# JohnsonLabJanelia/laserCalib

Hardware: AMD Instinct MI355X
Metric: LM iters/sec and residual+Jacobian Mobs/s at 16 cams x 50k points (higher is better)
Workload: dtype f32; 1 GPU; 16 cams x 50000 points per GPU, full visibility, 11-parameter cameras (800000 obs per GPU, 800000 total), full on-device Schur-complement LM iteration; cams=16, points_per_gpu=50000, camera_parameters=11, observations_total=800000, parallelism=points sharded x1, cameras replicated, collectives=none

## Files before the change

lasercalib_amd/csrc/sba_chol_blocked.hpp:

```cpp
#pragma once
#include "sba_lm_kernels.hpp"

namespace SBA_NS {

constexpr int CB = 16;
constexpr int CLD = 17;
constexpr int CBS = CB * CLD;
constexpr int CHOLB_THREADS = 512;
constexpr int CHOLB_LDS_THREADS = 512;
constexpr int CHOLB_MAX_NB = 11;

__device__ inline int cb_off(int r, int c) { return (r * (r + 1) / 2 + c) * CBS; }

__device__ inline double readlane_f64(double v, int src) {
  const int lo = __builtin_amdgcn_readlane(__double2loint(v), src);
  const int hi = __builtin_amdgcn_readlane(__double2hiint(v), src);
  return __hiloint2double(hi, lo);
}
__device__ inline double rsqrt_nr(double x) {
  const double y = __builtin_amdgcn_rsq(x);
  return y * (1.5 - 0.5 * x * y * y);
}

template <bool NEWTON = true>
// ... 206 lines not shown
  for (int ks = 0; ks < 4; ++ks) pp = Mfma<S>::mma(pt[ks], pt[ks], pp);
#pragma unroll
  for (int rg = 0; rg < 4; ++rg) d[rg] -= pp[rg];
#pragma unroll
  for (int rg = 0; rg < 4; ++rg) Pblk[(lane & 15) * L::LD + Mfma<S>::row_of(lane, rg)] = pt[rg];
#pragma unroll
  for (int rg = 0; rg < 4; ++rg) Dt[Mfma<S>::row_of(lane, rg) * L::LD + (lane & 15)] = d[rg];
  __builtin_amdgcn_wave_barrier();
}

template <int MAXNB> struct CholbShared {
  int fail;
  short rc[MAXNB * (MAXNB + 1) / 2];
  double dd[MAXNB * CB];
  double x[MAXNB * CB];
};
template <int MAXNB> struct CholbPre {
  static constexpr int BPR = CHOLB_LDS_THREADS / 128;
  static constexpr int U0 = (MAXNB + BPR - 1) / BPR;
  static constexpr int NREM = MAXNB * (MAXNB - 1) / 2;
  static constexpr int TREM = CHOLB_LDS_THREADS - 64;
  static constexpr int U1_ALL = (NREM * 128 + TREM - 1) / TREM;
  static constexpr int U1 = U1_ALL < 16 ? U1_ALL : 16;
};

template <typename S, bool NEWTON, bool PREFETCHED, int MAXNB, typename L = CholLay<S>>
__device__ __forceinline__ bool cholb_core(unsigned char* __restrict__ smem, CholbShared<MAXNB>& sh, const double* __restrict__ E, const int n,
                                           double (&c0)[CholbPre<MAXNB>::U0][2], double (&c1)[CholbPre<MAXNB>::U1][2], const int (&rc1)[CholbPre<MAXNB>::U1],
                                           const S tau, long long* __restrict__ dbg, int& nstamp) {
#define CHOL_STAMP() do { if (dbg && threadIdx.x == 0) dbg[nstamp] = clock64(); ++nstamp; } while (0)
  using Pre = CholbPre<MAXNB>;
  constexpr int BPR = Pre::BPR, U0 = Pre::U0, TREM = Pre::TREM, U1 = Pre::U1;
  constexpr bool F32 = std::is_same<S, float>::value;
  const int tid = threadIdx.x, lane = tid & 63, wid = tid >> 6;
  const int nb = (n + CB - 1) / CB;
  const int n16 = nb * CB;
  const int nblk = nb * (nb + 1) / 2;
  S* Lb = reinterpret_cast<S*>(smem);
  S* s_y = Lb + nblk * L::BS;
  S* s_a0 = s_y + n16;
  const int s4 = tid >> 7, ii0 = (tid >> 3) & 15, jp0 = tid & 7;
  auto fix = [&](int I, int J, double& v0, double& v1) {
    if (I >= n || J >= n) v0 = (I == J) ? 1.0 : 0.0;
    if (I >= n || J + 1 >= n) v1 = (I == J + 1) ? 1.0 : 0.0;
  };
  if (tid < n16) s_y[tid] = (S)sh.x[tid];
  if constexpr (PREFETCHED) {
#pragma unroll
    for (int u = 0; u < U0; ++u) fix((BPR * u + s4) * CB + ii0, 2 * jp0, c0[u][0], c0[u][1]);
    {
      const int ii = ii0, jp = jp0;
#pragma unroll
      for (int u = 0; u < U0; ++u) {
        const int r = BPR * u + s4;
        if (r < nb) {
          const int I = r * CB + ii, J = 2 * jp;
          S* dst = Lb + L::off(r, 0) + ii * L::LD + J;
          const double v0 = c0[u][0] + ((I == J && I < n) ? sh.dd[I] : 0.0), v1 = c0[u][1] + ((I == J + 1 && I < n) ? sh.dd[I] : 0.0);
          dst[0] = (S)v0;
          dst[1] = (S)v1;
          if (F32 && I == J) s_a0[I] = (S)v0;
          if (F32 && I == J + 1) s_a0[I] = (S)v1;
        }
      }
    }
    __syncthreads();
    CHOL_STAMP();
    if (wid > 0) {
#pragma unroll
      for (int u = 0; u < U1; ++u) {
// ... 165 lines not shown
        const S* col = Lb + L::off(b, tid >> 4) + (tid & 15);
        S s0 = 0, s1 = 0;
#pragma unroll
        for (int i = 0; i < CB; i += 2) { s0 += col[i * L::LD] * s_y[b * CB + i]; s1 += col[(i + 1) * L::LD] * s_y[b * CB + i + 1]; }
        s_y[tid] -= s0 + s1;
      }
      __syncthreads();
    }
    if (tid < n16) sh.x[tid] = (double)s_y[tid];
  }
  __syncthreads();
  CHOL_STAMP();
  return fail;
#undef CHOL_STAMP
}

template <typename T, int MAXNB = CHOLB_MAX_NB, int LD32 = 20>
__global__ __launch_bounds__(CHOLB_LDS_THREADS) void k_cholesky_blocked(
    const double* __restrict__ E , int C,
    LMState* __restrict__ st, double* __restrict__ D2c, const ParamSets<T> ps,
    double* __restrict__ delta_c, int n_sys ,
    const int32_t* __restrict__ tie ,
    const int32_t* __restrict__ first ,
    long long* __restrict__ dbg , int use_f32, float tau32) {
  extern __shared__ __align__(16) unsigned char smem[];
  constexpr bool PIV_NEWTON = !std::is_same<T, float>::value;
  const int n = n_sys;
  const int tid = threadIdx.x, lane = tid & 63, wid = tid >> 6;
  const double* rhs = E + (size_t)n * n;
  const double* dU = rhs + n;
  const double* gct = dU + n;
  const bool pair_ok = (n & 1) == 0;
  using Pre = CholbPre<MAXNB>;
  using L32 = CholLay<float, LD32>;
  constexpr int BPR = Pre::BPR, U0 = Pre::U0, TREM = Pre::TREM, U1 = Pre::U1;
  double c0[U0][2];
  const int nlast = n - 1;
  auto addr = [&](int I, int J) { return E + (size_t)min(I, nlast) * n + min(J, nlast - 1 + (pair_ok ? 0 : 1)); };
  const int s4 = tid >> 7, ii0 = (tid >> 3) & 15, jp0 = tid & 7;
  const int tclamp = min(tid, nlast);
  if (pair_ok) {
#pragma unroll
    for (int u = 0; u < U0; ++u) {
      const double2 t = *reinterpret_cast<const double2*>(addr((BPR * u + s4) * CB + ii0, 2 * jp0));
      c0[u][0] = t.x; c0[u][1] = t.y;
    }
  } else {
#pragma unroll
    for (int u = 0; u < U0; ++u) {
      const double* q = addr((BPR * u + s4) * CB + ii0, 2 * jp0);
      c0[u][0] = q[0]; c0[u][1] = q[(2 * jp0 + 1 < n) ? 1 : 0];
    }
  }
  double in_d = D2c[tclamp], in_u = dU[tclamp], in_r = rhs[tclamp];
  const double my_g = (tid < n) ? gct[tid] : 0.0;
  double c1[U1][2];
  int rc1[U1];
  {
    const int nb_ = (n + CB - 1) / CB;
    const int last = (nb_ * (nb_ + 1) / 2 - nb_) * 128 - 1;
    int cc = 1, base = 0;
#pragma unroll
    for (int u = 0; u < U1; ++u) {
      const int e = min(max(tid - 64, 0) + TREM * u, last);
      const int k = e >> 7;
      while (k >= base + (nb_ - cc) && cc < nb_) { base += nb_ - cc; ++cc; }
      rc1[u] = ((cc + (k - base)) << 8) | cc;
      const int I = (cc + (k - base)) * CB + ((e >> 3) & 15), J = cc * CB + 2 * (e & 7);
      if (pair_ok) {
        const double2 t = *reinterpret_cast<const double2*>(addr(I, J));
        c1[u][0] = t.x; c1[u][1] = t.y;
      } else {
        const double* q = addr(I, J);
        c1[u][0] = q[0]; c1[u][1] = q[(J + 1 < n) ? 1 : 0];
      }
    }
  }
  if (st->status >= 0) return;
  const int cur_ = ps_cur(ps, st);
  const double* __restrict__ cams = ps.cams[cur_];
  double* __restrict__ cams_new = ps.cams[cur_ ^ 1];
// ... 13 lines not shown
  const double my_xs = (tid < n) ? cams[first ? first[tid] : tid] : 0.0;

  if (tid < nblk) {
    int r = 0;
    while ((r + 1) * (r + 2) / 2 <= tid) ++r;
    sh.rc[tid] = (short)((r << 8) | (tid - r * (r + 1) / 2));
  }
  if (tid == 0) { sh.fail = 0; st->cost = E[(size_t)n * n + 3 * n]; }
  if (tid < n16) {
    double dd = 0;
    if (tid >= n) in_r = 0;
    if (tid < n) {
      double d = in_d;
      if (fresh) { d = fmax(d, in_u); D2c[tid] = d; }
      dd = lam * fmax_pos(d);
    }
    sh.x[tid] = in_r;
    sh.dd[tid] = dd;
  }
  __syncthreads();
  bool fail;
  if constexpr (MAXNB > CHOLB_MAX_NB) {
    static_assert(std::is_same<T, float>::value, "the 16-block-row kernel exists for the fp32 engine only");
    fail = cholb_core<float, false, true, MAXNB, L32>(smem, sh, E, n, c0, c1, rc1, tau32, dbg, nstamp);
    if (tid == 0) { st->chol_retry = fail ? 1 : 0; if (fail) st->chol_f64_retries += 1; }
    if (fail) return;
  } else if constexpr (std::is_same<T, float>::value) {
    if (use_f32) {
      fail = cholb_core<float, false, true, MAXNB, L32>(smem, sh, E, n, c0, c1, rc1, tau32, dbg, nstamp);
      if (fail) {
        __syncthreads();
        if (tid == 0) sh.fail = 0;
        __syncthreads();
        fail = cholb_core<double, true, false, MAXNB>(smem, sh, E, n, c0, c1, rc1, 0.0, dbg, nstamp);
        if (tid == 0) atomicAdd(&st->chol_f64_retries, 1);
      }
    } else {
      fail = cholb_core<double, PIV_NEWTON, true, MAXNB>(smem, sh, E, n, c0, c1, rc1, 0.0, dbg, nstamp);
    }
  } else {
    fail = cholb_core<double, PIV_NEWTON, true, MAXNB>(smem, sh, E, n, c0, c1, rc1, 0.0, dbg, nstamp);
  }
  double pred = 0, dx2 = 0, x2 = 0, gm = 0;
  __shared__ double s_cnew[CHOLB_LDS_THREADS];
  if (tid < ncam) {
    const double d = fail ? 0.0 : sh.x[tie ? tie[tid] : tid];
    delta_c[tid] = d;
    cams_new[tid] = my_cam + d;
    s_cnew[tid] = my_cam + d;
  }
  if (tid < n) {
    const double d = fail ? 0.0 : sh.x[tid];
    pred = 0.5 * d * (sh.dd[tid] * d - my_g);
    dx2 = d * d;
    x2 = my_xs * my_xs;
    gm = fabs(my_g);
  }
  pred = wave_sum(pred); dx2 = wave_sum(dx2); x2 = wave_sum(x2); gm = wave_max(gm);
  if (lane == 0) { s_scr[0][wid] = pred; s_scr[1][wid] = dx2; s_scr[2][wid] = x2; s_scr[3][wid] = gm; }
  __syncthreads();
  if (tid == 0) {
    double p = 0, d2 = 0, xx = 0, g = 0;
    for (int w = 0; w < CHOLB_LDS_THREADS / 64; ++w) { p += s_scr[0][w]; d2 += s_scr[1][w]; xx += s_scr[2][w]; g = fmax(g, s_scr[3][w]); }
    st->pred_c = p; st->dx2_c = d2; st->x2_c = xx; st->gmax_c = g;
// ... 206 lines not shown
```

lasercalib_amd/csrc/sba_engine.hpp:

```cpp
#pragma once
#include "sba_common.hpp"
#include "sba_lm_kernels.hpp"
#include "sba_chol_blocked.hpp"
#include "sba_chol_ll.hpp"
#include "sba_chol_big.hpp"
#include "sba_sq_kernels.hpp"
#include "sba_schur_wide.hpp"
#include "sba_schur_f64.hpp"
#include "sba_ipc.hpp"
#include "sba_covariance.hpp"
#include "sba_triangulate.hpp"
#include "sba_layout.hpp"

namespace SBA_NS {
using namespace sba_host;

constexpr int MAX_CAMS = 128;

struct Knobs {
  bool no_dense = false;
  bool no_fused64 = false;
  bool no_wide = false;
  bool wide_pw2 = false;
  bool chol_ll = true, chol_ll_all = false;
  bool chol_f32 = true;
  float chol_f32_tau = 1.1920929e-7f;
  bool chol_big_dag = true;
  int chol_big_min_n = 209;
  bool decide_kernel = false;
  bool schur_scan = false;
  bool no_bf3_pairs = false;
  double dense_min_vis = 0.0;
  bool schur_debug = false;
  int schur_debug_skip = 0;
  bool chol_debug = false;
  bool upload_debug = false;
  bool solve_debug = false;
  long long ipc_timeout_ticks = IPC_TIMEOUT_TICKS;
  bool ipc_allow_cached = false;
};

inline Knobs read_knobs() {
  Knobs k;
  auto set = [](const char* name) { return getenv(name) != nullptr; };
  k.no_dense = set("SBA_NO_DENSE");
  k.no_fused64 = set("SBA_NO_FUSED64");
  k.no_wide = set("SBA_NO_WIDE");
  k.wide_pw2 = set("SBA_WIDE_PW2");
  k.decide_kernel = set("SBA_DECIDE_KERNEL");
  k.schur_scan = set("SBA_SCHUR_SCAN");
  k.no_bf3_pairs = set("SBA_NO_BF3_PAIRS");
  k.chol_debug = set("SBA_CHOL_DEBUG");
  k.upload_debug = set("SBA_UPLOAD_DEBUG");
  k.solve_debug = set("SBA_SOLVE_DEBUG");
  k.ipc_allow_cached = set("SBA_IPC_ALLOW_CACHED");
  if (const char* e = getenv("SBA_CHOL")) { k.chol_ll = std::string(e) != "blocked"; k.chol_ll_all = std::string(e) == "ll"; }
  if (const char* e = getenv("SBA_CHOL_F32")) k.chol_f32 = atoi(e) != 0;
  if (const char* e = getenv("SBA_CHOL_F32_TAU")) { char* end = nullptr; const double v = strtod(e, &end); if (end != e && v >= 0 && v < 1) k.chol_f32_tau = (float)v; }
  if (const char* e = getenv("SBA_CHOL_BIG")) k.chol_big_dag = std::string(e) != "launches";
  if (const char* e = getenv("SBA_CHOL_BIG_MIN_N")) {
    char* end = nullptr;
    const long v = strtol(e, &end, 10);
    if (end != e && *end == 0 && v >= 0) k.chol_big_min_n = (int)std::min<long>(v, CS_MAX_NB * CB);
  }
  if (const char* e = getenv("SBA_DENSE_MIN_VIS")) { char* end = nullptr; const double v = strtod(e, &end); if (end != e && v >= 0 && v <= 1) k.dense_min_vis = v; }
  if (const char* e = getenv("SBA_SCHUR_DEBUG")) { k.schur_debug = true; k.schur_debug_skip = std::max(0, atoi(e) - 1); }
  if (const char* e = getenv("SBA_IPC_TIMEOUT_S")) {
    char* end = nullptr;
    const double sec = strtod(e, &end);
    if (end != e && sec > 0 && sec < 3600) k.ipc_timeout_ticks = (long long)(sec * 1e8);
  }
  return k;
}

struct Layout {
  int C, N;
  int64_t M;
  bool dense, masked_ok, grp_indexed;
  int ngroups, npairs;
  int ncu;
// ... 122 lines not shown
  bool has_w = false;
  bool identity_perm = true;
  bool dense = false;
  bool masked_ok = false;
  DevBuf<uint16_t> vis_mask;
  DevBuf<uint16_t> grp_mask;
  DevBuf<int32_t> grp_start;
  bool grp_indexed = false;
  DevBuf<double> gdpart;
  std::vector<int64_t> perm;
  int nblk = 0, nchunk = 0, ngroups = 0, npairs = 0;
  int n = 0;
  Knobs kn;
  Route rt;

  DevBuf<T2> uv_pm, uv_cm;
  DevBuf<T> w_pm, w_cm;
  DevBuf<int32_t> ci_pm, pi_pm, pt_start, blk_pt, pi_cm, chunk_cam, chunk_begin, chunk_end, cam_chunk_start;
  DevBuf<int32_t> pair_ga, pair_gb;
  DevBuf<int4> blk_desc;
  DevBuf<double> cams[2], pts[2];
  DevBuf<T> ptsT[2], campre[2];
  int cur = 0;
  DevBuf<double> V, gp, D2p, D2c, U, gc, Upart, bpart, E_own, scal_own, delta_c, cost_part, gmax_part, trial_part;
  DevBuf<T> slabs, pfac;
  DevBuf<T2> r_pm;
  DevBuf<T> Jc_pm, Jp_pm;
  DevBuf<LMState> d_state_buf;
  struct { LMState* p = nullptr; } d_state;
  int st_slot = 0;
  bool pending_decide = false;
  const double* pend_scal = nullptr;
  int pend_ranks = 1;
  DevBuf<double> gmax_alt;
  double* gmax_cur = nullptr;
  DevBuf<sba_lm_iter_log> d_log;
  int log_read = 0;
  int cur_at_begin = 0;
  LMState* h_state = nullptr;
  sba_lm_opts opts{};
  bool lm_active = false;
  DevBuf<double> chol_sol, chol_work, chol_W, chol_Minv, chol_Ld, chol_yv;
  DevBuf<int> chol_info;
  unsigned chol_epoch = 0;
  DevBuf<unsigned> chol_dag_flags;
  DevBuf<double> chol_Mimg;
// ... 419 lines not shown
      hipLaunchKernelGGL(k_group_index, dim3((N + 255) / 256), dim3(256), 0, stream, ci_pm.p, pt_start.p, N, ngroups, grp_mask.p,
                         grp_start.p, up_flag.p);
      int flag = 1;
      HIPCHK(hipMemcpyAsync(&flag, up_flag.p, sizeof(int), hipMemcpyDeviceToHost, stream));
      up_sync();
      grp_indexed = (flag == 0);
    }
    int ncu = 256;
    hipDeviceProp_t prop;
    if (ngroups > 1 && hipGetDeviceProperties(&prop, device) == hipSuccess && prop.multiProcessorCount > 0) ncu = prop.multiProcessorCount;
    rt = plan_route<T>(Layout{C, N, M, dense, masked_ok, grp_indexed, ngroups, npairs, ncu}, kn);
    const int ksplit = rt.ksplit;

    for (int b = 0; b < 2; ++b) {
      cams[b].alloc((size_t)C * NCP); pts[b].alloc((size_t)N * 3);
      ptsT[b].alloc((size_t)N * 3); campre[b].alloc((size_t)C * CAMPRE);
    }
    pfac.alloc((size_t)std::max(N, 1) * PF);
    V.alloc((size_t)N * 6); gp.alloc((size_t)N * 3); D2p.alloc((size_t)N * 3); D2c.alloc(n);
    U.alloc((size_t)C * NCP * NCP); gc.alloc(n); Upart.alloc((size_t)std::max(1, nchunk) * 256);
    bpart.alloc(std::max((size_t)ngroups * ksplit * GROUP_ROWS, rt.fused_wide ? (size_t)ksplit * WIDE_ROWS : (size_t)0));
    slabs.alloc(std::max((size_t)npairs * ksplit * GROUP_TILES * GROUP_TILES * 256, rt.fused_wide ? (size_t)ksplit * WIDE_SLOTS * 256 : (size_t)0));
    E_own.alloc((size_t)n * n + 3 * n + 1); scal_own.alloc(NSCAL); delta_c.alloc(n);
    const int nres_blocks = (int)((M + PM_BLOCK - 1) / PM_BLOCK);
    const int nlinp = rt.nlinp;
    if (dev_general) has_vis_mask = (C <= GROUP_CAMS);
    else {
      has_vis_mask = nodup && !vmask.empty();
      if (has_vis_mask) vis_mask.upload(vmask, stream);
    }
    if (rt.fused_ok) gdpart.alloc((size_t)ksplit * 2 * (rt.fused_wide ? WIDE_ROWS : GROUP_ROWS));
    if (rt.pairs_fold_u) gdpart.alloc((size_t)ngroups * ksplit * 2 * GROUP_ROWS);
    cost_part.alloc((size_t)std::max(std::max(std::max(std::max(nblk, nres_blocks), ksplit), nlinp), 1)); gmax_part.alloc(std::max(std::max(std::max(nblk, ksplit), nlinp), 1)); gmax_alt.alloc(std::max(std::max(std::max(nblk, ksplit), nlinp), 1));
    trial_part.alloc((size_t)4 * std::max(std::max(nblk, rt.nbs_dense), 1));
    up_lap("allocations + H2D enqueue");
    up_sync();
    up_lap("H2D completion");
    uploaded = true;
    cur = 0;
    set_params(cams_h, pts_h);
    ++up_rep.stream_syncs;
    up_lap("parameters");
    up_rep.route = dev_dense ? SBA_ROUTE_DEVICE_DENSE : dev_general ? SBA_ROUTE_DEVICE_GENERAL : SBA_ROUTE_HOST;
    up_rep.dense = dense; up_rep.masked = masked_ok; up_rep.group_indexed = grp_indexed; up_rep.identity_perm = identity_perm;
    up_rep.n_blocks = nblk; up_rep.n_chunks = nchunk;
    up_rep.seconds_total = std::chrono::duration<double>(std::chrono::steady_clock::now() - up_begin).count();
// ... 729 lines not shown
    pending_decide = false;
    gmax_cur = gmax_part.p;
    lm_active = true;
    if (!std::isfinite(c0)) { err = "Residuals are not finite in the initial point."; return SBA_ERR_NONFINITE; }
    return SBA_OK;
  }

  int lm_linearize() override {
    if (!lm_active) { err = "sba_lm_begin has not been called"; return SBA_ERR_STATE; }
    poll_clean = false;
    if (!bf3_path()) flush_decide();
    if (sq_mode()) { launch_sq_linearize(d_state.p); return SBA_OK; }
    if (fused()) return SBA_OK;
    if (!lin_pts()) {
      prof_begin(KP_LINP);
      launch_linearize_points(d_state.p);
      prof_end(KP_LINP);
    }
    if (h_state->free_cams && !rt.pairs_fold_u) { prof_begin(KP_LINC); launch_linearize_cams(d_state.p); prof_end(KP_LINC); }
    return SBA_OK;
  }

  int lm_form_reduced(double* E) override { return form_reduced(E, nullptr); }
  int form_reduced(double* E, double* Pk) {
    if (!lm_active) { err = "sba_lm_begin has not been called"; return SBA_ERR_STATE; }
    poll_clean = false;
    if (!bf3_path()) flush_decide();
    if (sq_mode()) {
      if (opts.mode == SBA_MODE_CAMS_ONLY_SQ)
        hipLaunchKernelGGL(k_sq_pack_cams, dim3(64), dim3(256), 0, stream, sq_16.p, C, d_state.p, E);
      return SBA_OK;
    }
    if (h_state->free_cams) {
      prof_begin(KP_SCHUR);
      launch_schur();
      prof_end(KP_SCHUR);
    }
    prof_begin(KP_REDUCE);
    {
      const int fc = (int)h_state->free_cams;
      const bool wide = fused() && rt.fused_wide;
      const int ntw = wide_ntw(C);
      const int nt_launch = wide ? ntw * (ntw + 1) / 2 : npairs == 1 ? GROUP_TILES * (GROUP_TILES + 1) / 2 : GROUP_TILES * GROUP_TILES;
      const int np_arg = wide ? 1 : npairs;
      const int nblocks = (fc ? 4 * nt_launch * np_arg + (n + 15) / 16 : 0) + 1;
      const int emajor_mode = wide ? 3 : ((fused() && sizeof(T) == 4) || pairs_bf3()) ? 1 : 0;
      hipLaunchKernelGGL(k_build_exchange<T>, dim3(nblocks), dim3(1024), 0, stream, slabs.p, bpart.p, rt.ksplit, pair_ga.p,
                         pair_gb.p, np_arg, U.p, gc.p, cost_part.p, n_lin_parts(), C, fc, E, d_state.p,
                         (fused() || rt.pairs_fold_u) ? gdpart.p : (const double*)nullptr, Pk, emajor_mode, nt_launch);
    }
    prof_end(KP_REDUCE);
    return SBA_OK;
  }

  void launch_chol_big(double* Esys, int n_sys, bool tied, CholRoute route) {
    const int npad = cholbig_npad(n_sys), nbr = npad / BB, nbx = (n_sys + BB - 1) / BB;
    if (chol_W.n < (size_t)npad * npad) {
      chol_W.alloc((size_t)npad * npad); chol_Minv.alloc((size_t)nbr * BB * BB); chol_Ld.alloc((size_t)nbr * BB * BB);
      chol_yv.alloc(2 * (size_t)npad);
      std::vector<long long> empty(2 * (size_t)npad, CHOLBIG_X_EMPTY);
      HIPCHK(hipMemcpyAsync(chol_yv.p, empty.data(), empty.size() * sizeof(long long), hipMemcpyHostToDevice, stream));
      sync();
    }
    if (chol_sol.n < (size_t)n_sys) { chol_sol.alloc(n_sys); chol_info.alloc(1); }
    const size_t lds = (size_t)CHOLBIG_LDS_BLOCKS * CBS * sizeof(double);
    const bool dag = route != CholRoute::BIG_LAUNCHES, dag32 = route == CholRoute::BIG_DAG_F32;
    if (dag) {
      if (chol_dag_flags.n == 0) { chol_dag_flags.alloc(choldag_nflags(CHOLDAG_MAX_NBR)); chol_dag_flags.zero(stream); }
      if (chol_Mimg.n == 0) chol_Mimg.alloc((size_t)CHOLDAG_MAX_NBR * choldag_img<double>());
      if (chol_debug) { chol_dbg.alloc(8 * (CHOLDAG_MAX_NBR + 1)); chol_dbg.zero(stream); }
      const dim3 grid(1 + nbr * (nbr + 1) / 2);
      if (dag32)
// ... 8 lines not shown
        fprintf(stderr, "[chol_dag%s, the walker, x10 ns: wait for W(c,c-1), W(c,c) | load | panel | downdate | factor+inverse | image stored | flag]\n", dag32 ? " on f32 lanes" : "");
        for (int cc = 0; cc < nbr; ++cc) {
          const long long* v = sv.data() + 8 * cc;
          fprintf(stderr, "  c=%2d at %6lld:", cc, v[4] - sv[0]);
          if (cc > 0) fprintf(stderr, " wait %4lld | load %4lld | panel %4lld | downdate %4lld |", v[1] - sv[8 * (cc - 1) + 7], v[2] - v[1], v[3] - v[2], v[4] - v[3]);
          fprintf(stderr, " factor %4lld | image %4lld | flag %4lld | column %5lld\n", v[5] - v[4], v[6] - v[5], v[7] - v[6], cc > 0 ? v[7] - sv[8 * (cc - 1) + 7] : v[7] - v[0]);
        }
        chol_debug = false;
      }
    } else {
      hipLaunchKernelGGL(k_chol_big_prepare, dim3(nbr * (nbr + 1) / 2), dim3(256), 0, stream, Esys, n_sys, d_state.p, D2c.p,
                         chol_W.p, npad, chol_info.p);
      for (int j = 0; j < nbr; ++j) {
        const int q = nbr - 1 - j;
        hipLaunchKernelGGL(k_chol_big_step, dim3(std::max(1, q * (q + 1) / 2)), dim3(CHOLBIG_THREADS), lds, stream, chol_W.p, npad, j,
                           chol_Minv.p, chol_Ld.p, chol_info.p, d_state.p);
      }
    }
    hipLaunchKernelGGL(k_chol_big_back_all<T>, dim3(nbx), dim3(256), 0, stream, (const void*)chol_W.p, npad, n_sys, chol_Ld.p, chol_Minv.p,
                       chol_yv.p, ++chol_epoch, chol_sol.p, chol_info.p, d_state.p, dag ? (const void*)chol_Mimg.p : (const void*)nullptr,
                       dag32 ? 1 : 0, Esys, C, D2c.p, ps_lm(), delta_c.p, tied ? tie_map.p : nullptr, tied ? tie_first.p : nullptr);
  }

  int lm_solve_trial(double* E, double* scal) override {
    if (!lm_active) { err = "sba_lm_begin has not been called"; return SBA_ERR_STATE; }
    poll_clean = false;
    if (opts.mode == SBA_MODE_TRANSFORM_SQ) {
      hipLaunchKernelGGL(k_sq_solve12, dim3(1), dim3(64), 0, stream, sq_16.p, d_state.p, tsets());
      launch_sq_trial();
      return SBA_OK;
    }
    if (h_state->free_cams) {
      prof_begin(KP_CHOL);
      const bool tied = (opts.mode == SBA_MODE_SHARED_INTR);
      const int n_sys = tied ? n_tied : n;
      double* Esys = E;
      if (tied) {
        hipLaunchKernelGGL(k_tie_system, dim3(n_tied), dim3(256), 0, stream, E, n, n_tied, tie_pre_start.p, tie_pre_idx.p,
                           E_tied.p, d_state.p);
        Esys = E_tied.p;
      }
      const int32_t* tie = tied ? tie_map.p : nullptr;
      const int32_t* first = tied ? tie_first.p : nullptr;
      const int nb = (n_sys + CB - 1) / CB;
      const CholRoute route = chol_route<T>(n_sys, n, kn, card_shared);
      switch (route) {
        case CholRoute::LL:
        case CholRoute::LL_F32: {
          if (chol_work.n < (size_t)nb * (nb + 1) / 2 * CB * CB) chol_work.alloc((size_t)CLL_MAX_NB * (CLL_MAX_NB + 1) / 2 * CB * CB);
          if (chol_debug && chol_dbg.n < 128) { chol_dbg.alloc(128); chol_dbg.zero(stream); }
          if constexpr (sizeof(T) == 4) {
            if (route == CholRoute::LL_F32) {
              if (nb <= 14) {
                const size_t lds32 = ((size_t)(nb * (nb + 1) / 2) * CB * 20 + 2 * (size_t)nb * CB) * sizeof(float);
                hipLaunchKernelGGL((k_cholesky_blocked<T, 16, 20>), dim3(1), dim3(CHOLB_LDS_THREADS), lds32, stream, Esys, C, d_state.p, D2c.p,
                                   ps_lm(), delta_c.p, n_sys, tie, first, (long long*)nullptr, 1, kn.chol_f32_tau);
              } else {
                const size_t lds32 = ((size_t)(nb * (nb + 1) / 2) * CB * 17 + 2 * (size_t)nb * CB) * sizeof(float);
                hipLaunchKernelGGL((k_cholesky_blocked<T, 16, 17>), dim3(1), dim3(CHOLB_LDS_THREADS), lds32, stream, Esys, C, d_state.p, D2c.p,
                                   ps_lm(), delta_c.p, n_sys, tie, first, (long long*)nullptr, 1, kn.chol_f32_tau);
              }
            }
          }
          hipLaunchKernelGGL(k_cholesky_ll<T>, dim3(1), dim3(CLL_THREADS), CLL_LDS_BYTES, stream, Esys, C, d_state.p, D2c.p,
                             ps_lm(), delta_c.p, n_sys, tie, first, chol_work.p, chol_debug ? chol_dbg.p : nullptr,
                             route == CholRoute::LL_F32 ? 1 : 0);
          if (chol_debug) {
            const std::vector<long long> st = read_stamps(chol_dbg, 128);
            if (nb > 6) {
              const long long x0 = st[2 + 2 * 3], y0 = st[3 + 2 * 3];
              fprintf(stderr, "[chol_ll step 3, cycles after the step's barrier, per wave] X done:");
              for (int w = 0; w < 8; ++w) fprintf(stderr, " %lld", st[64 + w] - x0);
              fprintf(stderr, " | Y done:");
              for (int w = 0; w < 8; ++w) fprintf(stderr, " %lld", st[72 + w] - y0);
              fprintf(stderr, "\n[chol_ll back substitution, block row 5] x done (per wave, from wave 0's):");
              for (int w = 0; w < 8; ++w) fprintf(stderr, " %lld", st[80 + w] - st[80]);
              fprintf(stderr, " | barrier passed %lld | update done:", st[96] - st[80]);
              for (int w = 0; w < 8; ++w) fprintf(stderr, " %lld", st[88 + w] - st[96]);
              fprintf(stderr, " | barrier passed %lld\n", st[97] - st[96]);
            }
            fprintf(stderr, "[chol_ll stamps, cycles] setup %lld  chol0 %lld |", st[1] - st[0], st[2] - st[1]);
            for (int j = 0; j < nb; ++j) fprintf(stderr, " X%d %lld Y%d %lld |", j, st[3 + 2 * j] - st[2 + 2 * j], j, st[4 + 2 * j] - st[3 + 2 * j]);
            fprintf(stderr, " backsub %lld  epilogue %lld  total %lld\n", st[3 + 2 * nb] - st[2 + 2 * nb], st[4 + 2 * nb] - st[3 + 2 * nb], st[4 + 2 * nb] - st[0]);
            chol_debug = false;
          }
          break;
        }
        case CholRoute::BLOCKED: {
          const size_t lds = ((size_t)(nb * (nb + 1) / 2) * CBS + 2 * (size_t)nb * CB) * sizeof(double);
          if (chol_debug && chol_dbg.n == 0) { chol_dbg.alloc(64); }
          hipLaunchKernelGGL(k_cholesky_blocked<T>, dim3(1), dim3(CHOLB_LDS_THREADS), lds, stream, Esys, C, d_state.p, D2c.p,
                             ps_lm(), delta_c.p, n_sys, tie, first, chol_debug ? chol_dbg.p : nullptr, (sizeof(T) == 4 && kn.chol_f32) ? 1 : 0,
                             kn.chol_f32_tau);
          if (chol_debug) {
            const std::vector<long long> st = read_stamps(chol_dbg, 64);
            fprintf(stderr, "[chol stamps, cycles] load %lld  chol0 %lld |", st[1] - st[0], st[2] - st[1]);
            for (int j = 0; j < nb; ++j) fprintf(stderr, " B%d %lld C%d %lld |", j, st[3 + 2 * j] - st[2 + 2 * j], j, st[4 + 2 * j] - st[3 + 2 * j]);
            fprintf(stderr, " backsub %lld  epilogue %lld  total %lld\n", st[3 + 2 * nb] - st[2 + 2 * nb], st[4 + 2 * nb] - st[3 + 2 * nb], st[4 + 2 * nb] - st[0]);
            fprintf(stderr, "[chol C0, cycles after B0's barrier, per wave]");
            for (int w = 0; w < CHOLB_LDS_THREADS / 64; ++w) fprintf(stderr, " %lld", st[40 + w] - st[3]);
            fprintf(stderr, "\n");
            chol_debug = false;
          }
          break;
        }
        case CholRoute::STREAM: {
          if (chol_sol.n < (size_t)n_sys) { chol_sol.alloc(n_sys); chol_info.alloc(1); }
          if (chol_work.n < (size_t)nb * (nb + 1) / 2 * CB * CB) chol_work.alloc((size_t)nb * (nb + 1) / 2 * CB * CB);
          const size_t fixed = ((size_t)nb * CBS + (size_t)nb * CB) * sizeof(double);
          const int scap = std::min(64, std::max(nb, (int)((150 * 1024 - fixed) / (CBS * sizeof(double)))));
          const size_t lds = fixed + (size_t)scap * CBS * sizeof(double);
          if (chol_debug && chol_dbg.n == 0) chol_dbg.alloc(64);
          hipLaunchKernelGGL(k_chol_prepare, dim3((n_sys + 255) / 256), dim3(256), 0, stream, Esys, n_sys, d_state.p, D2c.p, chol_sol.p);
          hipLaunchKernelGGL(k_cholesky_stream, dim3(1), dim3(CHOLB_THREADS), lds, stream, Esys, n_sys, chol_work.p, chol_sol.p,
                             chol_info.p, d_state.p, scap, chol_debug ? chol_dbg.p : nullptr);
          if (chol_debug) {
            const std::vector<long long> st = read_stamps(chol_dbg, 8);
            fprintf(stderr, "[chol_stream cycles] update %lld  factor %lld  solve %lld  write-back %lld  back-substitution %lld\n", st[0], st[1], st[2], st[3], st[4]);
            chol_debug = false;
          }
          hipLaunchKernelGGL(k_chol_epilogue<T>, dim3(1), dim3(1024), 0, stream, Esys, C, n_sys, d_state.p, D2c.p, ps_lm(), delta_c.p,
                             chol_sol.p, chol_info.p, tie, first);
          break;
        }
// ... 157 lines not shown
    } else {
      for (int i = 0; i < n; ++i) gmax = std::max(gmax, std::fabs(gch[i]));
    }
    if (rep) {
      const LMState& s = *h_state;
      rep->cost = cost; rep->initial_cost = initial_cost; rep->optimality = gmax; rep->step_norm = s.step_norm;
      rep->lambda = s.lam; rep->nfev = s.nfev; rep->njev = s.njev; rep->iterations = s.iter; rep->accepted = s.n_accepted;
      rep->status = s.status < 0 ? 0 : s.status;
      rep->reserved = s.chol_f64_retries;
    }
    lm_active = false;
    return SBA_OK;
  }

  int run_loop(const sba_lm_opts* o, int32_t& status, int32_t& iters) {
    int rc = SBA_OK;
    while (status < 0) {
      const int pbatch = multi() ? 2 : (bf3_path() && !kn.decide_kernel ? 2 : 1);
      int batch = prof_on ? pbatch : BATCH;
      if (o->max_iter > 0) batch = std::min(std::max(1, o->max_iter - iters), prof_on ? pbatch : 64);
      for (int b = 0; b < batch; ++b) {
        lm_linearize();
        if (!multi()) {
          lm_form_reduced(E_own.p);
          lm_solve_trial(E_own.p, nullptr);
          lm_decide_async(nullptr, 1);
        } else if (ipc_on) {
          const bool fc = h_state->free_cams != 0;
          const unsigned long long s0 = ++ipc_seq[0];
          const size_t sys_off = ipc_L.sys_slot(n, (int)(s0 & 1));
          form_reduced(E_own.p, ipc_mine + sys_off);
          ipc_publish(0, s0, d_state.p);
          ipc_gate(0, s0, d_state.p, 0, 0, nullptr);
          hipLaunchKernelGGL(k_ipc_sum_system, dim3(fc ? std::min(1024, (n * n + 255) / 256) : 1), dim3(256), 0, stream, ipc_ptrs.p, comm_n,
                             sys_off, n, (int)fc, E_own.p, d_state.p);
          const unsigned long long s1 = ++ipc_seq[1];
          const size_t sc_off = ipc_L.scal_slot((int)(s1 & 1));
          lm_solve_trial(E_own.p, ipc_mine + sc_off);
          ipc_publish(1, s1, d_state.p);
          ipc_gate(1, s1, d_state.p, sc_off, NSCAL, sc_all.p);
          lm_decide_async(sc_all.p, comm_n);
        } else {
          if (xpack.n < exch_packed_size(n)) xpack.alloc(exch_packed_size(n));
          form_reduced(E_own.p, xpack.p);
          const bool fc = h_state->free_cams != 0;
          double* xb = fc ? xpack.p : xpack.p + exch_packed_size(n) - 1;
          RCCLCHK(Rccl::get().all_reduce(xb, xb, fc ? exch_packed_size(n) : 1, Rccl::kFloat64, Rccl::kSum, comm, stream));
          hipLaunchKernelGGL(k_unpack_exchange, dim3(fc ? std::min(1024, (n * n + 255) / 256) : 1), dim3(256), 0, stream, xpack.p, n,
// ... 200 lines not shown
```

lasercalib_amd/csrc/sba_lm_kernels.hpp:

```cpp
#pragma once
#include <cstddef>
#include "sba_kernels.hpp"

namespace SBA_NS {

constexpr int CHOL_THREADS = 1024;
constexpr int CHOL_LDS_MAX_N = 176;

__host__ __device__ inline size_t exch_packed_index(int n, int i, int j) { return (size_t)i * n - (size_t)i * (i - 1) / 2 + (size_t)(j - i); }
__host__ __device__ inline size_t exch_packed_size(int n) { return (size_t)n * (n + 1) / 2 + 3 * (size_t)n + 1; }

template <typename T>
__global__ __launch_bounds__(1024) void k_build_exchange(
    const T* __restrict__ slabs, const double* __restrict__ bpart, int ksplit, const int32_t* __restrict__ pair_ga,
    const int32_t* __restrict__ pair_gb, int npairs, const double* __restrict__ U, const double* __restrict__ gc,
    const double* __restrict__ cost_part, int n_cost_part, int C, int free_cams, double* __restrict__ E,
    const LMState* __restrict__ st,
    const double* __restrict__ gdpart ,
    double* __restrict__ Pk = nullptr ,
    int emajor_mode = 0 ,
    int nt_launch = GROUP_TILES * GROUP_TILES ) {
  using M_ = Mfma<T>;
  constexpr int EPB = 64, NG = 1024 / EPB, BPT = 256 / EPB;
  __shared__ double s_p[NG][EPB];
  const int st_status = st->status;
  __shared__ double scr[16];
  constexpr int NT = GROUP_TILES * GROUP_TILES;
  const int n = C * NCP;
  const int tile_blocks = free_cams ? BPT * nt_launch * npairs : 0;
  const int row_blocks = free_cams ? (n + 15) / 16 : 0;
  const int g = threadIdx.x / EPB, l16 = threadIdx.x & (EPB - 1);
  int bid = blockIdx.x;
  if (bid < tile_blocks) {
    const bool wide = emajor_mode == 3;
    const int pair = wide ? 0 : bid / (BPT * nt_launch);
    const int rem = bid - pair * BPT * nt_launch;
    const int t = rem / BPT, part = rem - t * BPT;
    const int ga = pair_ga[pair], gb = pair_gb[pair];
    const bool diag = wide || (ga == gb);
    const int ntw = wide_ntw(C);
    const int ntile = wide ? ntw * (ntw + 1) / 2 : diag ? (GROUP_TILES * (GROUP_TILES + 1)) / 2 : NT;
    if (t >= ntile) return;
    int R, Tc;
    if (wide) wide_tile_rc(ntw, t, R, Tc);
// ... 25 lines not shown
      for (; k + 3 * NG < ksplit; k += 4 * NG) {
        s0 += (double)src[(size_t)k * stride];
        s1 += (double)src[(size_t)(k + NG) * stride];
        s2 += (double)src[(size_t)(k + 2 * NG) * stride];
        s3 += (double)src[(size_t)(k + 3 * NG) * stride];
      }
      for (; k < ksplit; k += NG) s0 += (double)src[(size_t)k * stride];
    }
    const int ci_ = i / NCP, cj_ = j / NCP;
    s_p[g][l16] = (s0 + s1) + (s2 + s3);
    __syncthreads();
    if (st_status >= 0) return;
    if (g == 0 && i < n && j < n) {
      double s = 0;
#pragma unroll
      for (int q = 0; q < NG; ++q) s += s_p[q][l16];
      double v = -s;
      if (!gdpart && ci_ == cj_) v += U[(size_t)ci_ * NCP * NCP + (i - ci_ * NCP) * NCP + (j - cj_ * NCP)];
      const bool sym_tile = diag && R == Tc;
      if (!emajor) {
        E[(size_t)i * n + j] = v;
        if (!sym_tile) E[(size_t)j * n + i] = v;
        if (Pk && i <= j) Pk[exch_packed_index(n, i, j)] = v;
      } else if (!sym_tile || i <= j) {
        E[(size_t)i * n + j] = v;
        E[(size_t)j * n + i] = v;
        if (Pk) Pk[exch_packed_index(n, i < j ? i : j, i < j ? j : i)] = v;
      }
    }
    return;
  }
  bid -= tile_blocks;
  double* rhs = E + (size_t)n * n;
  double* dU = rhs + n;
  double* gv = dU + n;
  if (bid < row_blocks) {
    constexpr int RB = 16, RG = 1024 / RB;
    __shared__ double s_r[3][RG][RB];
    const int lr = threadIdx.x & (RB - 1), gr = threadIdx.x / RB;
    const int i = bid * RB + lr;
    double b0 = 0, g0 = 0, d0 = 0;
    if (i < n) {
      const bool wide = emajor_mode == 3;
      const int rstride = wide ? WIDE_ROWS : GROUP_ROWS;
      const int grp = wide ? 0 : i / GROUP_ROWS, rho = i - grp * GROUP_ROWS;
      const double* src = bpart + (size_t)grp * ksplit * GROUP_ROWS + rho;
      if (gdpart) {
        const double* gs_ = gdpart + (size_t)grp * ksplit * 2 * GROUP_ROWS + rho;
        for (int k = gr; k < ksplit; k += RG) {
          b0 += src[(size_t)k * rstride];
// ... 554 lines not shown
```

Measured before the change: 7356 Mobs/s (observations x LM iterations per second, whole job).

## Write fp32 blocked-lower image in exchange build and load it in Cholesky

The exchange-matrix build kernel now also writes an fp32 copy of the reduced camera system, already laid out as 16x16 lower-triangular blocks. The blocked Cholesky kernel then loads whole blocks as float4 per wave from this image, instead of gathering fp64 pairs from the dense row-major E and converting them. The diagonal is rebuilt from E's diagonal plus damping, and padding is pre-initialised to identity on the host. This is meant to cut the load and convert phase of the single-block Cholesky. In exchange it adds extra scattered stores in the build kernel and a new buffer.

New measurement: 7494 Mobs/s (observations x LM iterations per second, whole job), median of 6. +1.9%, better.

```diff
diff --git a/lasercalib_amd/csrc/sba_chol_blocked.hpp b/lasercalib_amd/csrc/sba_chol_blocked.hpp
--- a/lasercalib_amd/csrc/sba_chol_blocked.hpp
+++ b/lasercalib_amd/csrc/sba_chol_blocked.hpp
@@ -252,16 +252,26 @@
   static constexpr int TREM = CHOLB_LDS_THREADS - 64;
   static constexpr int U1_ALL = (NREM * 128 + TREM - 1) / TREM;
   static constexpr int U1 = U1_ALL < 16 ? U1_ALL : 16;
+  static constexpr int PU0 = (MAXNB + CHOLB_LDS_THREADS / 64 - 1) / (CHOLB_LDS_THREADS / 64);
+  static constexpr int PU1 = (NREM + CHOLB_LDS_THREADS / 64 - 2) / (CHOLB_LDS_THREADS / 64 - 1);
+};
+template <int MAXNB> struct CholbImg {
+  const float* img;
+  float4 p0[CholbPre<MAXNB>::PU0];
+  float4 p1[CholbPre<MAXNB>::PU1];
+  int rc1[CholbPre<MAXNB>::PU1];
+  double e_dg;
 };
 
 template <typename S, bool NEWTON, bool PREFETCHED, int MAXNB, typename L = CholLay<S>>
 __device__ __forceinline__ bool cholb_core(unsigned char* __restrict__ smem, CholbShared<MAXNB>& sh, const double* __restrict__ E, const int n,
                                            double (&c0)[CholbPre<MAXNB>::U0][2], double (&c1)[CholbPre<MAXNB>::U1][2], const int (&rc1)[CholbPre<MAXNB>::U1],
-                                           const S tau, long long* __restrict__ dbg, int& nstamp) {
+                                           const CholbImg<MAXNB>& pk, const S tau, long long* __restrict__ dbg, int& nstamp) {
 #define CHOL_STAMP() do { if (dbg && threadIdx.x == 0) dbg[nstamp] = clock64(); ++nstamp; } while (0)
   using Pre = CholbPre<MAXNB>;
   constexpr int BPR = Pre::BPR, U0 = Pre::U0, TREM = Pre::TREM, U1 = Pre::U1;
   constexpr bool F32 = std::is_same<S, float>::value;
+  constexpr int NWV = CHOLB_LDS_THREADS / 64;
   const int tid = threadIdx.x, lane = tid & 63, wid = tid >> 6;
   const int nb = (n + CB - 1) / CB;
   const int n16 = nb * CB;
@@ -275,7 +285,35 @@
     if (I >= n || J + 1 >= n) v1 = (I == J + 1) ? 1.0 : 0.0;
   };
   if (tid < n16) s_y[tid] = (S)sh.x[tid];
-  if constexpr (PREFETCHED) {
+  if (F32 && PREFETCHED && pk.img) {
+    if constexpr (F32 && PREFETCHED) {
+      const int ii = lane >> 2, q4 = lane & 3;
+      auto put = [&](int br, int bc, float4 v) {
+        if (br == bc) {
+          const float d = s_a0[br * CB + ii];
+          if (q4 == (ii >> 2)) { const int cq = ii & 3; v.x = cq == 0 ? d : v.x; v.y = cq == 1 ? d : v.y; v.z = cq == 2 ? d : v.z; v.w = cq == 3 ? d : v.w; }
+        }
+        float* dst = Lb + L::off(br, bc) + ii * L::LD + 4 * q4;
+        if constexpr (L::LD % 4 == 0) *reinterpret_cast<float4*>(dst) = v;
+        else { dst[0] = v.x; dst[1] = v.y; dst[2] = v.z; dst[3] = v.w; }
+      };
+      if (tid < n16) s_a0[tid] = (tid < n) ? (float)(pk.e_dg + sh.dd[tid]) : 1.0f;
+      __builtin_amdgcn_wave_barrier();
+#pragma unroll
+      for (int u = 0; u < Pre::PU0; ++u) {
+        const int r = NWV * u + wid;
+        if (r < nb) put(r, 0, pk.p0[u]);
+      }
+      __syncthreads();
+      CHOL_STAMP();
+      if (wid > 0) {
+#pragma unroll
+        for (int u = 0; u < Pre::PU1; ++u) {
+          if ((wid - 1) + (NWV - 1) * u < nblk - nb) put(pk.rc1[u] >> 8, pk.rc1[u] & 255, pk.p1[u]);
+        }
+      }
+    }
+  } else if constexpr (PREFETCHED) {
 #pragma unroll
     for (int u = 0; u < U0; ++u) fix((BPR * u + s4) * CB + ii0, 2 * jp0, c0[u][0], c0[u][1]);
     {
@@ -487,7 +525,8 @@
     double* __restrict__ delta_c, int n_sys ,
     const int32_t* __restrict__ tie ,
     const int32_t* __restrict__ first ,
-    long long* __restrict__ dbg , int use_f32, float tau32) {
+    long long* __restrict__ dbg , int use_f32, float tau32,
+    const float* __restrict__ img = nullptr ) {
   extern __shared__ __align__(16) unsigned char smem[];
   constexpr bool PIV_NEWTON = !std::is_same<T, float>::value;
   const int n = n_sys;
@@ -504,7 +543,20 @@
   auto addr = [&](int I, int J) { return E + (size_t)min(I, nlast) * n + min(J, nlast - 1 + (pair_ok ? 0 : 1)); };
   const int s4 = tid >> 7, ii0 = (tid >> 3) & 15, jp0 = tid & 7;
   const int tclamp = min(tid, nlast);
-  if (pair_ok) {
+  CholbImg<MAXNB> pk;
+  if (!std::is_same<T, float>::value || !(MAXNB > CHOLB_MAX_NB || use_f32)) img = nullptr;
+  pk.img = img;
+  pk.e_dg = 0.0;
+  if (img) {
+    const int nb_ = (n + CB - 1) / CB;
+    const float4* im4 = reinterpret_cast<const float4*>(img);
+#pragma unroll
+    for (int u = 0; u < Pre::PU0; ++u) {
+      const int r = min((CHOLB_LDS_THREADS / 64) * u + wid, nb_ - 1);
+      pk.p0[u] = im4[(size_t)(r * (r + 1) / 2) * 64 + lane];
+    }
+    pk.e_dg = E[(size_t)tclamp * n + tclamp];
+  } else if (pair_ok) {
 #pragma unroll
     for (int u = 0; u < U0; ++u) {
       const double2 t = *reinterpret_cast<const double2*>(addr((BPR * u + s4) * CB + ii0, 2 * jp0));
@@ -521,7 +573,22 @@
   const double my_g = (tid < n) ? gct[tid] : 0.0;
   double c1[U1][2];
   int rc1[U1];
-  {
+  if (img) {
+   if (wid > 0) {
+    const int nb_ = (n + CB - 1) / CB, nblk_ = nb_ * (nb_ + 1) / 2;
+    const float4* im4 = reinterpret_cast<const float4*>(img);
+    const int w1 = __builtin_amdgcn_readfirstlane(wid - 1);
+    int cc = 1, base = 0;
+#pragma unroll
+    for (int u = 0; u < Pre::PU1; ++u) {
+      const int k = max(min(w1 + (CHOLB_LDS_THREADS / 64 - 1) * u, nblk_ - nb_ - 1), 0);
+      while (k >= base + (nb_ - cc) && cc < nb_) { base += nb_ - cc; ++cc; }
+      const int r = cc + (k - base);
+      pk.rc1[u] = (r << 8) | cc;
+      pk.p1[u] = im4[(size_t)min(r * (r + 1) / 2 + cc, nblk_ - 1) * 64 + lane];
+    }
+   }
+  } else {
     const int nb_ = (n + CB - 1) / CB;
     const int last = (nb_ * (nb_ + 1) / 2 - nb_) * 128 - 1;
     int cc = 1, base = 0;
@@ -581,24 +648,24 @@
   bool fail;
   if constexpr (MAXNB > CHOLB_MAX_NB) {
     static_assert(std::is_same<T, float>::value, "the 16-block-row kernel exists for the fp32 engine only");
-    fail = cholb_core<float, false, true, MAXNB, L32>(smem, sh, E, n, c0, c1, rc1, tau32, dbg, nstamp);
+    fail = cholb_core<float, false, true, MAXNB, L32>(smem, sh, E, n, c0, c1, rc1, pk, tau32, dbg, nstamp);
     if (tid == 0) { st->chol_retry = fail ? 1 : 0; if (fail) st->chol_f64_retries += 1; }
     if (fail) return;
   } else if constexpr (std::is_same<T, float>::value) {
     if (use_f32) {
-      fail = cholb_core<float, false, true, MAXNB, L32>(smem, sh, E, n, c0, c1, rc1, tau32, dbg, nstamp);
+      fail = cholb_core<float, false, true, MAXNB, L32>(smem, sh, E, n, c0, c1, rc1, pk, tau32, dbg, nstamp);
       if (fail) {
         __syncthreads();
         if (tid == 0) sh.fail = 0;
         __syncthreads();
-        fail = cholb_core<double, true, false, MAXNB>(smem, sh, E, n, c0, c1, rc1, 0.0, dbg, nstamp);
+        fail = cholb_core<double, true, false, MAXNB>(smem, sh, E, n, c0, c1, rc1, pk, 0.0, dbg, nstamp);
         if (tid == 0) atomicAdd(&st->chol_f64_retries, 1);
       }
     } else {
-      fail = cholb_core<double, PIV_NEWTON, true, MAXNB>(smem, sh, E, n, c0, c1, rc1, 0.0, dbg, nstamp);
+      fail = cholb_core<double, PIV_NEWTON, true, MAXNB>(smem, sh, E, n, c0, c1, rc1, pk, 0.0, dbg, nstamp);
     }
   } else {
-    fail = cholb_core<double, PIV_NEWTON, true, MAXNB>(smem, sh, E, n, c0, c1, rc1, 0.0, dbg, nstamp);
+    fail = cholb_core<double, PIV_NEWTON, true, MAXNB>(smem, sh, E, n, c0, c1, rc1, pk, 0.0, dbg, nstamp);
   }
   double pred = 0, dx2 = 0, x2 = 0, gm = 0;
   __shared__ double s_cnew[CHOLB_LDS_THREADS];
diff --git a/lasercalib_amd/csrc/sba_engine.hpp b/lasercalib_amd/csrc/sba_engine.hpp
--- a/lasercalib_amd/csrc/sba_engine.hpp
+++ b/lasercalib_amd/csrc/sba_engine.hpp
@@ -25,6 +25,7 @@
   bool chol_ll = true, chol_ll_all = false;
   bool chol_f32 = true;
   float chol_f32_tau = 1.1920929e-7f;
+  bool chol_packed = true;
   bool chol_big_dag = true;
   int chol_big_min_n = 209;
   bool decide_kernel = false;
@@ -56,6 +57,7 @@
   k.ipc_allow_cached = set("SBA_IPC_ALLOW_CACHED");
   if (const char* e = getenv("SBA_CHOL")) { k.chol_ll = std::string(e) != "blocked"; k.chol_ll_all = std::string(e) == "ll"; }
   if (const char* e = getenv("SBA_CHOL_F32")) k.chol_f32 = atoi(e) != 0;
+  if (const char* e = getenv("SBA_CHOL_PACKED")) k.chol_packed = atoi(e) != 0;
   if (const char* e = getenv("SBA_CHOL_F32_TAU")) { char* end = nullptr; const double v = strtod(e, &end); if (end != e && v >= 0 && v < 1) k.chol_f32_tau = (float)v; }
   if (const char* e = getenv("SBA_CHOL_BIG")) k.chol_big_dag = std::string(e) != "launches";
   if (const char* e = getenv("SBA_CHOL_BIG_MIN_N")) {
@@ -224,6 +226,7 @@
   DevBuf<double> cams[2], pts[2];
   DevBuf<T> ptsT[2], campre[2];
   int cur = 0;
+  DevBuf<float> chol_img;
   DevBuf<double> V, gp, D2p, D2c, U, gc, Upart, bpart, E_own, scal_own, delta_c, cost_part, gmax_part, trial_part;
   DevBuf<T> slabs, pfac;
   DevBuf<T2> r_pm;
@@ -689,6 +692,16 @@
     bpart.alloc(std::max((size_t)ngroups * ksplit * GROUP_ROWS, rt.fused_wide ? (size_t)ksplit * WIDE_ROWS : (size_t)0));
     slabs.alloc(std::max((size_t)npairs * ksplit * GROUP_TILES * GROUP_TILES * 256, rt.fused_wide ? (size_t)ksplit * WIDE_SLOTS * 256 : (size_t)0));
     E_own.alloc((size_t)n * n + 3 * n + 1); scal_own.alloc(NSCAL); delta_c.alloc(n);
+    if (sizeof(T) == 4 && kn.chol_f32 && kn.chol_packed && !kn.chol_ll_all && n <= CLL_MAX_NB * CB) {
+      const int nbi = (n + CB - 1) / CB;
+      std::vector<float> ident((size_t)nbi * (nbi + 1) / 2 * CB * CB, 0.0f);
+      for (int r = 0; r < nbi; ++r)
+        for (int i = 0; i < CB; ++i) ident[((size_t)r * (r + 1) / 2 + r) * CB * CB + i * CB + i] = 1.0f;
+      chol_img.upload(ident, stream);
+      sync();
+    } else {
+      chol_img.free();
+    }
     const int nres_blocks = (int)((M + PM_BLOCK - 1) / PM_BLOCK);
     const int nlinp = rt.nlinp;
     if (dev_general) has_vis_mask = (C <= GROUP_CAMS);
@@ -1464,7 +1477,7 @@
   }
 
   int lm_form_reduced(double* E) override { return form_reduced(E, nullptr); }
-  int form_reduced(double* E, double* Pk) {
+  int form_reduced(double* E, double* Pk, bool packed = false) {
     if (!lm_active) { err = "sba_lm_begin has not been called"; return SBA_ERR_STATE; }
     poll_clean = false;
     if (!bf3_path()) flush_decide();
@@ -1489,7 +1502,8 @@
       const int emajor_mode = wide ? 3 : ((fused() && sizeof(T) == 4) || pairs_bf3()) ? 1 : 0;
       hipLaunchKernelGGL(k_build_exchange<T>, dim3(nblocks), dim3(1024), 0, stream, slabs.p, bpart.p, rt.ksplit, pair_ga.p,
                          pair_gb.p, np_arg, U.p, gc.p, cost_part.p, n_lin_parts(), C, fc, E, d_state.p,
-                         (fused() || rt.pairs_fold_u) ? gdpart.p : (const double*)nullptr, Pk, emajor_mode, nt_launch);
+                         (fused() || rt.pairs_fold_u) ? gdpart.p : (const double*)nullptr, Pk, emajor_mode, nt_launch,
+                         packed ? chol_img.p : (float*)nullptr);
     }
     prof_end(KP_REDUCE);
     return SBA_OK;
@@ -1544,7 +1558,18 @@
                        dag32 ? 1 : 0, Esys, C, D2c.p, ps_lm(), delta_c.p, tied ? tie_map.p : nullptr, tied ? tie_first.p : nullptr);
   }
 
-  int lm_solve_trial(double* E, double* scal) override {
+  void print_cholb_stamps(int nb) {
+    const std::vector<long long> st = read_stamps(chol_dbg, 64);
+    fprintf(stderr, "[chol stamps, cycles] load %lld  chol0 %lld |", st[1] - st[0], st[2] - st[1]);
+    for (int j = 0; j < nb; ++j) fprintf(stderr, " B%d %lld C%d %lld |", j, st[3 + 2 * j] - st[2 + 2 * j], j, st[4 + 2 * j] - st[3 + 2 * j]);
+    fprintf(stderr, " backsub %lld  epilogue %lld  total %lld\n", st[3 + 2 * nb] - st[2 + 2 * nb], st[4 + 2 * nb] - st[3 + 2 * nb], st[4 + 2 * nb] - st[0]);
+    fprintf(stderr, "[chol C0, cycles after B0's barrier, per wave]");
+    for (int w = 0; w < CHOLB_LDS_THREADS / 64; ++w) fprintf(stderr, " %lld", st[40 + w] - st[3]);
+    fprintf(stderr, "\n");
+  }
+
+  int lm_solve_trial(double* E, double* scal) override { return solve_trial(E, scal, false); }
+  int solve_trial(double* E, double* scal, bool packed) {
     if (!lm_active) { err = "sba_lm_begin has not been called"; return SBA_ERR_STATE; }
     poll_clean = false;
     if (opts.mode == SBA_MODE_TRANSFORM_SQ) {
@@ -1564,6 +1589,7 @@
       }
       const int32_t* tie = tied ? tie_map.p : nullptr;
       const int32_t* first = tied ? tie_first.p : nullptr;
+      const float* img = (packed && !tied) ? chol_img.p : nullptr;
       const int nb = (n_sys + CB - 1) / CB;
       const CholRoute route = chol_route<T>(n_sys, n, kn, card_shared);
       switch (route) {
@@ -1573,15 +1599,17 @@
           if (chol_debug && chol_dbg.n < 128) { chol_dbg.alloc(128); chol_dbg.zero(stream); }
           if constexpr (sizeof(T) == 4) {
             if (route == CholRoute::LL_F32) {
+              long long* dbg32 = chol_debug ? chol_dbg.p : nullptr;
               if (nb <= 14) {
                 const size_t lds32 = ((size_t)(nb * (nb + 1) / 2) * CB * 20 + 2 * (size_t)nb * CB) * sizeof(float);
                 hipLaunchKernelGGL((k_cholesky_blocked<T, 16, 20>), dim3(1), dim3(CHOLB_LDS_THREADS), lds32, stream, Esys, C, d_state.p, D2c.p,
-                                   ps_lm(), delta_c.p, n_sys, tie, first, (long long*)nullptr, 1, kn.chol_f32_tau);
+                                   ps_lm(), delta_c.p, n_sys, tie, first, dbg32, 1, kn.chol_f32_tau, img);
               } else {
                 const size_t lds32 = ((size_t)(nb * (nb + 1) / 2) * CB * 17 + 2 * (size_t)nb * CB) * sizeof(float);
                 hipLaunchKernelGGL((k_cholesky_blocked<T, 16, 17>), dim3(1), dim3(CHOLB_LDS_THREADS), lds32, stream, Esys, C, d_state.p, D2c.p,
-                                   ps_lm(), delta_c.p, n_sys, tie, first, (long long*)nullptr, 1, kn.chol_f32_tau);
+                                   ps_lm(), delta_c.p, n_sys, tie, first, dbg32, 1, kn.chol_f32_tau, img);
               }
+              if (chol_debug) print_cholb_stamps(nb);
             }
           }
           hipLaunchKernelGGL(k_cholesky_ll<T>, dim3(1), dim3(CLL_THREADS), CLL_LDS_BYTES, stream, Esys, C, d_state.p, D2c.p,
@@ -1613,15 +1641,9 @@
           if (chol_debug && chol_dbg.n == 0) { chol_dbg.alloc(64); }
           hipLaunchKernelGGL(k_cholesky_blocked<T>, dim3(1), dim3(CHOLB_LDS_THREADS), lds, stream, Esys, C, d_state.p, D2c.p,
                              ps_lm(), delta_c.p, n_sys, tie, first, chol_debug ? chol_dbg.p : nullptr, (sizeof(T) == 4 && kn.chol_f32) ? 1 : 0,
-                             kn.chol_f32_tau);
+                             kn.chol_f32_tau, img);
           if (chol_debug) {
-            const std::vector<long long> st = read_stamps(chol_dbg, 64);
-            fprintf(stderr, "[chol stamps, cycles] load %lld  chol0 %lld |", st[1] - st[0], st[2] - st[1]);
-            for (int j = 0; j < nb; ++j) fprintf(stderr, " B%d %lld C%d %lld |", j, st[3 + 2 * j] - st[2 + 2 * j], j, st[4 + 2 * j] - st[3 + 2 * j]);
-            fprintf(stderr, " backsub %lld  epilogue %lld  total %lld\n", st[3 + 2 * nb] - st[2 + 2 * nb], st[4 + 2 * nb] - st[3 + 2 * nb], st[4 + 2 * nb] - st[0]);
-            fprintf(stderr, "[chol C0, cycles after B0's barrier, per wave]");
-            for (int w = 0; w < CHOLB_LDS_THREADS / 64; ++w) fprintf(stderr, " %lld", st[40 + w] - st[3]);
-            fprintf(stderr, "\n");
+            print_cholb_stamps(nb);
             chol_debug = false;
           }
           break;
@@ -1825,8 +1847,10 @@
       for (int b = 0; b < batch; ++b) {
         lm_linearize();
         if (!multi()) {
-          lm_form_reduced(E_own.p);
-          lm_solve_trial(E_own.p, nullptr);
+          const CholRoute croute = chol_route<T>(n, n, kn, card_shared);
+          const bool packed = chol_img.n != 0 && opts.mode == SBA_MODE_FULL && (croute == CholRoute::BLOCKED || croute == CholRoute::LL_F32);
+          form_reduced(E_own.p, nullptr, packed);
+          solve_trial(E_own.p, nullptr, packed);
           lm_decide_async(nullptr, 1);
         } else if (ipc_on) {
           const bool fc = h_state->free_cams != 0;
diff --git a/lasercalib_amd/csrc/sba_lm_kernels.hpp b/lasercalib_amd/csrc/sba_lm_kernels.hpp
--- a/lasercalib_amd/csrc/sba_lm_kernels.hpp
+++ b/lasercalib_amd/csrc/sba_lm_kernels.hpp
@@ -9,6 +9,11 @@
 
 __host__ __device__ inline size_t exch_packed_index(int n, int i, int j) { return (size_t)i * n - (size_t)i * (i - 1) / 2 + (size_t)(j - i); }
 __host__ __device__ inline size_t exch_packed_size(int n) { return (size_t)n * (n + 1) / 2 + 3 * (size_t)n + 1; }
+
+__device__ __forceinline__ void chol_img_store(float* __restrict__ img, int i, int j, double v) {
+  const int bi = i >> 4, bj = j >> 4;
+  if (bi >= bj) img[((bi * (bi + 1) / 2 + bj) << 8) + ((i & 15) << 4) + (j & 15)] = (float)v;
+}
 
 template <typename T>
 __global__ __launch_bounds__(1024) void k_build_exchange(
@@ -19,7 +24,8 @@
     const double* __restrict__ gdpart ,
     double* __restrict__ Pk = nullptr ,
     int emajor_mode = 0 ,
-    int nt_launch = GROUP_TILES * GROUP_TILES ) {
+    int nt_launch = GROUP_TILES * GROUP_TILES ,
+    float* __restrict__ img = nullptr ) {
   using M_ = Mfma<T>;
   constexpr int EPB = 64, NG = 1024 / EPB, BPT = 256 / EPB;
   __shared__ double s_p[NG][EPB];
@@ -91,10 +97,12 @@
         E[(size_t)i * n + j] = v;
         if (!sym_tile) E[(size_t)j * n + i] = v;
         if (Pk && i <= j) Pk[exch_packed_index(n, i, j)] = v;
+        if (img) { chol_img_store(img, i, j, v); if (!sym_tile) chol_img_store(img, j, i, v); }
       } else if (!sym_tile || i <= j) {
         E[(size_t)i * n + j] = v;
         E[(size_t)j * n + i] = v;
         if (Pk) Pk[exch_packed_index(n, i < j ? i : j, i < j ? j : i)] = v;
+        if (img) { chol_img_store(img, i, j, v); chol_img_store(img, j, i, v); }
       }
     }
     return;
```
